# TaceoLabs/collaborative-circom

Hardware: AMD Instinct MI355X
Metric: Groth16 constraints/sec (BN254, 2^22 R1CS), one REP3 party's prove (higher is better)
Workload: dtype u32; 1 GPU; synthetic R1CS 2^22 constraints-domain BN254, REP3 co-groth16 (configs[2]); num_constraints=4194302, domain_size=4194304, nnz=12582906, msm=8 G1 + 2 G2 of ~2^22 points, ntt=12

## Files before the change

collaborative-circom_amd/csrc/capi_internal.hpp:

```cpp
#pragma once
#include "common.hpp"
#include "launchers.hpp"
#include "curve.hpp"
#include "subgroup.hpp"
#include "host_ec64.hpp"
#include "ntt_kernels.hpp"
#include "plonk_kernels.hpp"

#include <cmath>
#include <chrono>
#include <map>
#include <set>
#include <mutex>
#include <vector>

using namespace cg;

hipError_t hip_malloc_flush(void** p, size_t bytes);
template <class T> hipError_t hip_malloc_flush(T** p, size_t bytes) { return hip_malloc_flush((void**)p, bytes); }

namespace cgi {

struct Arena {
    char* base = nullptr; size_t cap = 0, used = 0;
    void* take(size_t bytes) { void* p = base + used; used += align_up(bytes); return p; }
};

enum { TW_BITREV = 1, TW_NATURAL = 2 };
struct TwKey { int curve; int log_m; uint32_t gen[8]; int kind = 0;
    bool operator<(const TwKey& o) const { if (curve != o.curve) return curve < o.curve; if (log_m != o.log_m) return log_m < o.log_m; if (kind != o.kind) return kind < o.kind; return memcmp(gen, o.gen, sizeof gen) < 0; } };
struct CosetKey { TwKey k; uint32_t scale[8]; bool operator<(const CosetKey& o) const { if (k < o.k) return true; if (o.k < k) return false; return memcmp(scale, o.scale, sizeof scale) < 0; } };
struct CosetTables { void* lo; void* hi; int log_lo; };

enum { TAG_MSM = 0, TAG_NTT, TAG_VEC, TAG_SPMV, TAG_SORT, TAG_ACC_G1, TAG_ACC_G2, TAG_REDUCE, TAG_COUNT };
struct EvPair { hipEvent_t a, b; int tag; };

struct MsmFold { enum { WINDOWS = 0, PLAIN = 1, BITS = 2, GRID = 3 }; int kind = WINDOWS, c = 0, nsums = 0, log_l = 0, log_h = 0; uint32_t gc = 1, gr = 1; };

struct MsmTicket {
    bool live = false;
    int curve = 0, group = 0, k = 0, c = 0, nwin = 0;
    uint32_t* h_flags = nullptr; bool optimistic = false;
    const cg_bases* bases = nullptr; size_t offset = 0, n = 0; std::vector<const void*> scalars;
    int nsums = 0;
    MsmFold fold;
    void* h_pinned = nullptr; size_t pinned_bytes = 0;
    hipEvent_t done = nullptr;
};

}
using namespace cgi;


// ... 166 lines not shown
```

collaborative-circom_amd/csrc/capi_ntt.hip:

```cpp
#include "capi_internal.hpp"

namespace {
template <class Fr>
void host_pow_tables(const Fr& w, const Fr& first, int log_lo, size_t hi_n, std::vector<Fr>& lo, std::vector<Fr>& hi) {
    lo.resize((size_t)1 << log_lo); hi.resize(hi_n);
    Fr acc = first, step = Fr::one();
    for (size_t j = 0; j < lo.size(); j++) { lo[j] = acc; acc = acc * w; step = step * w; }
    Fr h = Fr::one();
    for (size_t j = 0; j < hi_n; j++) { hi[j] = h; h = h * step; }
}

struct SharedTwiddles { void* p; size_t bytes; int refs; uint64_t stamp; };
std::mutex g_tw_mu;
std::map<std::pair<int, TwKey>, SharedTwiddles> g_tw;
uint64_t g_tw_clock = 0;
void* shared_twiddles_acquire(int device, const TwKey& key) {
    std::lock_guard<std::mutex> l(g_tw_mu);
    auto it = g_tw.find({device, key});
    if (it == g_tw.end()) return nullptr;
    it->second.refs++; it->second.stamp = ++g_tw_clock;
    return it->second.p;
}
void* shared_twiddles_publish(int device, const TwKey& key, void* p, size_t bytes) {
    std::lock_guard<std::mutex> l(g_tw_mu);
// ... 4 lines not shown
}
}
void shared_twiddles_release(int device, const TwKey& key) {
    std::lock_guard<std::mutex> l(g_tw_mu);
    auto it = g_tw.find({device, key});
    if (it != g_tw.end() && it->second.refs > 0) it->second.refs--;
    for (;;) {
        size_t idle = 0; auto victim = g_tw.end();
        for (auto j = g_tw.begin(); j != g_tw.end(); ++j) if (j->second.refs == 0) { idle += j->second.bytes; if (victim == g_tw.end() || j->second.stamp < victim->second.stamp) victim = j; }
        if (idle <= ((size_t)1 << 30) || victim == g_tw.end()) break;
        hipFree(victim->second.p); g_tw.erase(victim);
    }
}
namespace {

template <class Fr> Fr mont32() { Fr c = Fr::one(); for (int i = 0; i < 5; i++) c = c + c; return c; }
template <class Fr> Fr inv_pow2(int log_m) {
    uint32_t e[Fr::N] = {0}; e[log_m / 32] = 1u << (log_m % 32);
    Fr nn; for (int i = 0; i < Fr::N; i++) nn.v[i] = e[i];
    return fp_inverse(nn.to_mont());
}

template <class Fr>
int get_twiddles_lazy(cg_ctx* ctx, int curve, int log_m, const Fr& w, bool natural, const void** out) {
    TwKey key; key.curve = curve; key.log_m = log_m; key.kind = natural ? TW_NATURAL : TW_BITREV; memcpy(key.gen, w.v, sizeof key.gen);
    auto it = ctx->twiddles.find(key);
    if (it != ctx->twiddles.end()) { *out = it->second; return 0; }
    if (void* shared = shared_twiddles_acquire(ctx->device, key)) { ctx->twiddles[key] = shared; *out = shared; return 0; }
    const size_t m = (size_t)1 << log_m;
    const int log_lo = std::min(11, std::max(0, log_m - 1));
    const size_t hi_n = std::max<size_t>(1, (m / 2) >> log_lo);
    std::vector<Fr> lo, hi;
    host_pow_tables(w, Fr::one(), log_lo, hi_n, lo, hi);
    Fr *d_lo = nullptr, *d_hi = nullptr; void* d_tw = nullptr;
    const size_t bytes = lazy29_bytes(std::max<size_t>(m / 2, 1));
    HIPCHK(hip_malloc_flush((void**)&d_lo, lo.size() * sizeof(Fr)));
    HIPCHK(hip_malloc_flush((void**)&d_hi, hi.size() * sizeof(Fr)));
    HIPCHK(hip_malloc_flush(&d_tw, bytes));
    HIPCHK(hipMemcpyAsync(d_lo, lo.data(), lo.size() * sizeof(Fr), hipMemcpyHostToDevice, ctx->stream));
    HIPCHK(hipMemcpyAsync(d_hi, hi.data(), hi.size() * sizeof(Fr), hipMemcpyHostToDevice, ctx->stream));
    {
        const int rc = natural ? launch_build_twiddles_lazy_natural<Fr>(ctx->stream, d_tw, m, d_lo, d_hi, log_lo, mont32<Fr>())
                               : launch_build_twiddles_lazy<Fr>(ctx->stream, d_tw, m, log_m, d_lo, d_hi, log_lo, mont32<Fr>());
        if (rc) return rc;
    }
    HIPCHK(hipStreamSynchronize(ctx->stream));
    HIPCHK(hipFree(d_lo)); HIPCHK(hipFree(d_hi));
    d_tw = shared_twiddles_publish(ctx->device, key, d_tw, bytes);
    ctx->twiddles[key] = d_tw;
    *out = d_tw;
    return 0;
}

template <class Fr>
int get_coset_tables(cg_ctx* ctx, int curve, int log_m, const Fr& g, const Fr& scale, CosetTables* out) {
    CosetKey key; key.k.curve = curve; key.k.log_m = log_m; memcpy(key.k.gen, g.v, sizeof key.k.gen); memcpy(key.scale, scale.v, sizeof key.scale);
    auto it = ctx->cosets.find(key);
    if (it != ctx->cosets.end()) { *out = it->second; return 0; }
    const size_t m = (size_t)1 << log_m;
    const int log_lo = std::min(11, log_m);
    const size_t hi_n = std::max<size_t>(1, m >> log_lo);
    std::vector<Fr> lo, hi;
    host_pow_tables(g, scale, log_lo, hi_n, lo, hi);
    CosetTables t; t.log_lo = log_lo;
    HIPCHK(hip_malloc_flush(&t.lo, lo.size() * sizeof(Fr)));
    HIPCHK(hip_malloc_flush(&t.hi, hi.size() * sizeof(Fr)));
    HIPCHK(hipMemcpy(t.lo, lo.data(), lo.size() * sizeof(Fr), hipMemcpyHostToDevice));
    HIPCHK(hipMemcpy(t.hi, hi.data(), hi.size() * sizeof(Fr), hipMemcpyHostToDevice));
    if (ctx->cosets.size() >= 64) {
        HIPCHK(hipStreamSynchronize(ctx->stream));
// ... 17 lines not shown
            int k = rest / np + (i < rest % np ? 1 : 0);
            plan.push_back({s0, k, tile_log - k});
            s0 += k;
        }
    }
    plan.push_back({s0, k_last, 0});
    return plan;
}

int ntt_lazy_tile() {
    static const int tile = [] { const char* e = tune_env("CG_NTT_TILE"); const int v = e ? atoi(e) : NTT_TILE_LOG_LAZY; return std::min(NTT_TILE_LOG, std::max(8, v)); }();
    return tile;
}

template <class Fr>
int ntt_run(cg_ctx* ctx, int curve, void* const* d_vecs, int k, size_t n, const Fr& gen, bool inverse, const Fr* coset, size_t arena_off) {
    const int log_m = log2_floor(n);
    if (((size_t)1 << log_m) != n) return fail(CG_ERR_ARG, "NTT length must be a power of two");
    if (k < 1 || k > NTT_MAX_VECS) return fail(CG_ERR_ARG, "k out of range");
    if (n == 1) return 0;
    if (!inverse && coset) return fail(CG_ERR_ARG, "coset_gen is only supported with inverse != 0");
    const Fr w = inverse ? fp_inverse(gen) : gen;
    const void* twl = nullptr;
    int rc = get_twiddles_lazy<Fr>(ctx, curve, log_m, w, false, &twl);
    if (rc) return rc;
    NttVecs data{}, tmp{};
    for (int j = 0; j < k; j++) { data.p[j] = d_vecs[j]; tmp.p[j] = ctx->ntt_arena.base + arena_off + (size_t)j * lazy29_bytes(n); }
    hipStream_t st = ctx->stream;
    bool first = true;
    for (const NttPass& p : ntt_plan(log_m, ntt_lazy_tile())) { rc = launch_ntt_ct_pass<Fr>(st, first, first ? data : tmp, tmp, k, n, log_m, p.s0, p.k, p.t, twl); if (rc) return rc; first = false; }
    const Fr scale32 = inverse ? mont32<Fr>() * inv_pow2<Fr>(log_m) : mont32<Fr>();
    CosetTables t;
    const Fr* d_scale = nullptr; const Fr* c_lo = nullptr; const Fr* c_hi = nullptr; int log_lo = 0;
    if (coset) { rc = get_coset_tables<Fr>(ctx, curve, log_m, *coset, scale32, &t); if (rc) return rc; c_lo = (const Fr*)t.lo; c_hi = (const Fr*)t.hi; log_lo = t.log_lo; }
    else { rc = get_coset_tables<Fr>(ctx, curve, 0, Fr::one(), scale32, &t); if (rc) return rc; d_scale = (const Fr*)t.lo; }
    return launch_bitrev_finish_lazy<Fr>(st, data, tmp, k, n, log_m, d_scale, c_lo, c_hi, log_lo);
}

template <class Fr>
int ntt_coset_pair_run(cg_ctx* ctx, int curve, void* const* d_vecs, int k, size_t n, const Fr& gen, const Fr& coset, size_t arena_off) {
    const int log_m = log2_floor(n);
    if (((size_t)1 << log_m) != n) return fail(CG_ERR_ARG, "NTT length must be a power of two");
    if (k < 1 || k > NTT_MAX_VECS) return fail(CG_ERR_ARG, "k out of range");
    if (n == 1) return 0;
    const void* tw_inv = nullptr; const void* tw_fwd = nullptr;
    int rc = get_twiddles_lazy<Fr>(ctx, curve, log_m, fp_inverse(gen), false, &tw_inv); if (rc) return rc;
    rc = get_twiddles_lazy<Fr>(ctx, curve, log_m, gen, true, &tw_fwd); if (rc) return rc;
    const Fr c32 = mont32<Fr>();
    CosetTables ct;
    rc = get_coset_tables<Fr>(ctx, curve, log_m, coset, c32 * inv_pow2<Fr>(log_m), &ct); if (rc) return rc;
    NttVecs data{}, tmp{};
    for (int j = 0; j < k; j++) { data.p[j] = d_vecs[j]; tmp.p[j] = ctx->ntt_arena.base + arena_off + (size_t)j * lazy29_bytes(n); }
    hipStream_t st = ctx->stream;
    const std::vector<NttPass> plan = ntt_plan(log_m, ntt_lazy_tile());
    bool first = true;
    for (const NttPass& p : plan) { rc = launch_ntt_ct_pass<Fr>(st, first, first ? data : tmp, tmp, k, n, log_m, p.s0, p.k, p.t, tw_inv); if (rc) return rc; first = false; }
    for (size_t i = plan.size(); i-- > 0;) {
        const NttPass& p = plan[i];
        rc = launch_ntt_dit_pass<Fr>(st, i + 1 == plan.size(), i == 0, data, tmp, k, n, log_m, p.s0, p.k, p.t, tw_fwd, (const Fr*)ct.lo, (const Fr*)ct.hi, ct.log_lo, c32);
        if (rc) return rc;
    }
    return 0;
}

}

extern "C" {
int32_t cg_ntt_dev(cg_ctx* ctx, int32_t curve, void* const* d_vecs, int32_t k, size_t n, const void* h_group_gen, int32_t inverse, const void* h_coset_gen) {
    if (!ctx || !d_vecs || !h_group_gen) return fail(CG_ERR_ARG, "null argument");
    HIPCHK(hipSetDevice(ctx->device));
    return with_fr(curve, [&](auto tag) -> int {
        typedef decltype(tag) Fr;
        Fr gen, cos; copy_in(gen, h_group_gen);
        if (h_coset_gen) copy_in(cos, h_coset_gen);
        if (n > 1) { int rc = ensure_ntt_arena(ctx, (size_t)k * lazy29_bytes(n)); if (rc) return rc; }
        StatScope ss(ctx, TAG_NTT);
        return ntt_run<Fr>(ctx, curve, d_vecs, k, n, gen, inverse != 0, h_coset_gen ? &cos : nullptr, 0);
    });
}
int32_t cg_ntt_coset_pair_dev(cg_ctx* ctx, int32_t curve, void* const* d_vecs, int32_t k, size_t n, const void* h_group_gen, const void* h_coset_gen) {
    if (!ctx || !d_vecs || !h_group_gen || !h_coset_gen) return fail(CG_ERR_ARG, "null argument");
    HIPCHK(hipSetDevice(ctx->device));
// ... 38 lines not shown
```

collaborative-circom_amd/csrc/fr_impl.hpp:

```cpp
#pragma once
#include "launchers.hpp"
#include "ntt_kernels.hpp"
#include "vec_kernels.hpp"
#include "plonk_kernels.hpp"
#include "r1cs_kernels.hpp"
#include "plonk_setup_kernels.hpp"
#include "msm_sort_kernels.hpp"

namespace cg {

template <class Fr> int launch_vec_binary(hipStream_t st, int op, Fr* out, const Fr* a, const Fr* b, size_t n) {
    if (!n) return 0;
    if (op == 0) hipLaunchKernelGGL((k_vec_binary<Fr, 0>), dim3(grid_for(n)), dim3(256), 0, st, out, a, b, n);
    else if (op == 1) hipLaunchKernelGGL((k_vec_binary<Fr, 1>), dim3(grid_for(n)), dim3(256), 0, st, out, a, b, n);
    else hipLaunchKernelGGL((k_vec_binary<Fr, 2>), dim3(grid_for(n)), dim3(256), 0, st, out, a, b, n);
    HIPCHK(hipGetLastError());
    return 0;
}
template <class Fr> int launch_rep3_mul_local(hipStream_t st, Fr* out, const Fr* aa, const Fr* ab, const Fr* ba, const Fr* bb, const Fr* mask, size_t n) {
    if (!n) return 0;
    hipLaunchKernelGGL((k_rep3_mul_local<Fr>), dim3(grid_for(n)), dim3(256), 0, st, out, aa, ab, ba, bb, mask, n);
    HIPCHK(hipGetLastError());
    return 0;
}
// ... 151 lines not shown
template <class Fr> int launch_plonk_sigma_labels(hipStream_t st, const uint32_t* prev, const Fr* wpow, int log_n, const Fr& k1, const Fr& k2, Fr* sigma) {
    hipLaunchKernelGGL((k_plonk_sigma_labels<Fr>), dim3(grid_for((size_t)3 << log_n)), dim3(256), 0, st, prev, wpow, log_n, k1, k2, sigma);
    HIPCHK(hipGetLastError());
    return 0;
}
template <class Fr> int launch_build_twiddles_lazy(hipStream_t st, void* tw, size_t m, int log_m, const Fr* lo, const Fr* hi, int log_lo, const Fr& c32) {
    if (m > 1) hipLaunchKernelGGL((k_build_twiddles_lazy<Fr>), dim3(grid_for(m / 2)), dim3(256), 0, st, tw, m / 2, log_m, lo, hi, log_lo, c32);
    HIPCHK(hipGetLastError());
    return 0;
}
template <class Fr> int launch_ntt_ct_pass(hipStream_t st, bool first, NttVecs src, NttVecs dst, int nvec, size_t n, int log_m, int s0, int k, int t, const void* tw) {
    static PerDeviceOnce attr_set;
    if (attr_set.pending()) {
        HIPCHK(hipFuncSetAttribute((const void*)k_ntt_ct_pass<Fr, true>, hipFuncAttributeMaxDynamicSharedMemorySize, 36 << NTT_TILE_LOG));
        HIPCHK(hipFuncSetAttribute((const void*)k_ntt_ct_pass<Fr, false>, hipFuncAttributeMaxDynamicSharedMemorySize, 36 << NTT_TILE_LOG));
        attr_set.mark();
    }
    const int E = 1 << (k + t);
    if (first) hipLaunchKernelGGL((k_ntt_ct_pass<Fr, true>), dim3((unsigned)(n / E), nvec), dim3(NTT_THREADS), (size_t)E * 36, st, src, dst, log_m, s0, k, t, tw);
    else hipLaunchKernelGGL((k_ntt_ct_pass<Fr, false>), dim3((unsigned)(n / E), nvec), dim3(NTT_THREADS), (size_t)E * 36, st, src, dst, log_m, s0, k, t, tw);
    HIPCHK(hipGetLastError());
    return 0;
}
template <class Fr> int launch_build_twiddles_lazy_natural(hipStream_t st, void* tw, size_t m, const Fr* lo, const Fr* hi, int log_lo, const Fr& c32) {
    if (m > 1) hipLaunchKernelGGL((k_build_twiddles_lazy_natural<Fr>), dim3(grid_for(m / 2)), dim3(256), 0, st, tw, m / 2, lo, hi, log_lo, c32);
    HIPCHK(hipGetLastError());
    return 0;
}
template <class Fr> int launch_ntt_dit_pass(hipStream_t st, bool first, bool last, NttVecs out, NttVecs tmp, int nvec, size_t n, int log_m, int s0, int k, int t, const void* tw,
                                            const Fr* c_lo, const Fr* c_hi, int log_lo, const Fr& c32) {
    static PerDeviceOnce attr_set;
    if (attr_set.pending()) {
        HIPCHK(hipFuncSetAttribute((const void*)k_ntt_dit_pass<Fr, true, true>, hipFuncAttributeMaxDynamicSharedMemorySize, 36 << NTT_TILE_LOG));
        HIPCHK(hipFuncSetAttribute((const void*)k_ntt_dit_pass<Fr, true, false>, hipFuncAttributeMaxDynamicSharedMemorySize, 36 << NTT_TILE_LOG));
        HIPCHK(hipFuncSetAttribute((const void*)k_ntt_dit_pass<Fr, false, true>, hipFuncAttributeMaxDynamicSharedMemorySize, 36 << NTT_TILE_LOG));
        HIPCHK(hipFuncSetAttribute((const void*)k_ntt_dit_pass<Fr, false, false>, hipFuncAttributeMaxDynamicSharedMemorySize, 36 << NTT_TILE_LOG));
        attr_set.mark();
    }
    const int E = 1 << (k + t);
    const dim3 grid((unsigned)(n / E), nvec); const size_t lds = (size_t)E * 36;
    if (first && last) hipLaunchKernelGGL((k_ntt_dit_pass<Fr, true, true>), grid, dim3(NTT_THREADS), lds, st, out, tmp, log_m, s0, k, t, tw, c_lo, c_hi, log_lo, c32);
    else if (first) hipLaunchKernelGGL((k_ntt_dit_pass<Fr, true, false>), grid, dim3(NTT_THREADS), lds, st, out, tmp, log_m, s0, k, t, tw, c_lo, c_hi, log_lo, c32);
    else if (last) hipLaunchKernelGGL((k_ntt_dit_pass<Fr, false, true>), grid, dim3(NTT_THREADS), lds, st, out, tmp, log_m, s0, k, t, tw, c_lo, c_hi, log_lo, c32);
    else hipLaunchKernelGGL((k_ntt_dit_pass<Fr, false, false>), grid, dim3(NTT_THREADS), lds, st, out, tmp, log_m, s0, k, t, tw, c_lo, c_hi, log_lo, c32);
    HIPCHK(hipGetLastError());
    return 0;
}
template <class Fr> int launch_bitrev_finish_lazy(hipStream_t st, NttVecs dst, NttVecs src, int nvec, size_t n, int log_m, const Fr* scale, const Fr* c_lo, const Fr* c_hi, int log_lo) {
    if (log_m >= 2 * BITREV_B_LAZY)
        hipLaunchKernelGGL((k_bitrev_finish_lazy<Fr>), dim3((unsigned)(n >> (2 * BITREV_B_LAZY)), nvec), dim3(256), 0, st, dst, src, log_m, scale, c_lo, c_hi, log_lo);
    else
        hipLaunchKernelGGL((k_bitrev_finish_lazy_small<Fr>), dim3(grid_for(n), nvec), dim3(256), 0, st, dst, src, log_m, scale, c_lo, c_hi, log_lo);
    HIPCHK(hipGetLastError());
    return 0;
}

inline bool msm_sort_use_partition(size_t n, int c, int nwin, int shared, bool any_size = false) {
    const size_t nbuckets = (size_t)(shared ? 1 : nwin) << (c - 1);
    const size_t nregions = (nbuckets + ((size_t)1 << PART_REGION_LOG) - 1) >> PART_REGION_LOG;
    return (any_size || (size_t)nwin * n >= ((size_t)1 << 21)) && nregions >= 8 && nregions <= PART_MAX_REGIONS;
}
template <class Fr> int msm_sort_launch(hipStream_t st, const Fr* d_scalars, size_t n, int c, int nwin, int shared, char* scratch, size_t scratch_bytes, MsmSortPtrs* out, hipEvent_t* evs,
                                        int force) {
    if (force != 0 && force != CG_MSM_PATH_GENERAL && force != CG_MSM_PATH_SMALL && force != CG_MSM_PATH_PARTITION) return fail(CG_ERR_ARG, "msm_sort_launch: not a path of the dense schedule");
    const size_t nbuckets = (size_t)(shared ? 1 : nwin) << (c - 1);
    size_t off = 0;
    auto take = [&](size_t bytes) { void* p = scratch + off; off += align_up(bytes); return p; };
// ... 119 lines not shown
    template decltype(launch_vec_gather_strided<Fr>) launch_vec_gather_strided<Fr>;                                        \
    template decltype(launch_vec_lincomb<Fr>) launch_vec_lincomb<Fr>;                                                      \
    template decltype(launch_shamir_share<Fr>) launch_shamir_share<Fr>;                                                    \
    template decltype(launch_plonk_r2_factors<Fr>) launch_plonk_r2_factors<Fr>;                                            \
    template decltype(launch_prefix_scan<Fr>) launch_prefix_scan<Fr>;                                                      \
    template decltype(launch_vec_inverse<Fr>) launch_vec_inverse<Fr>;                                                      \
    template decltype(launch_plonk_additions<Fr>) launch_plonk_additions<Fr>;                                              \
    template decltype(launch_plonk_r3_blind<Fr>) launch_plonk_r3_blind<Fr>;                                                \
    template decltype(launch_plonk_r3_perm<Fr>) launch_plonk_r3_perm<Fr>;                                                  \
    template decltype(launch_plonk_r3_gate<Fr>) launch_plonk_r3_gate<Fr>;                                                  \
    template decltype(launch_plonk_mul4_tail<Fr>) launch_plonk_mul4_tail<Fr>;                                              \
    template decltype(launch_plonk_r3_t<Fr>) launch_plonk_r3_t<Fr>;                                                        \
    template decltype(launch_plonk_r3_divide<Fr>) launch_plonk_r3_divide<Fr>;                                              \
    template decltype(launch_plonk_gate_check<Fr>) launch_plonk_gate_check<Fr>;                                            \
    template decltype(launch_vec_mismatch<Fr>) launch_vec_mismatch<Fr>;                                                    \
    template decltype(launch_spmv_csr<Fr>) launch_spmv_csr<Fr>;                                                            \
    template decltype(launch_r1cs_check<Fr>) launch_r1cs_check<Fr>;                                                        \
    template decltype(launch_qap_columns<Fr>) launch_qap_columns<Fr>;                                                      \
    template decltype(launch_plonk_gate_count<Fr>) launch_plonk_gate_count<Fr>;                                            \
    template decltype(launch_plonk_gate_emit<Fr>) launch_plonk_gate_emit<Fr>;                                              \
    template decltype(launch_plonk_sigma_labels<Fr>) launch_plonk_sigma_labels<Fr>;                                        \
    template decltype(launch_build_twiddles_lazy<Fr>) launch_build_twiddles_lazy<Fr>;                                      \
    template decltype(launch_ntt_ct_pass<Fr>) launch_ntt_ct_pass<Fr>;                                                      \
    template decltype(launch_build_twiddles_lazy_natural<Fr>) launch_build_twiddles_lazy_natural<Fr>;                      \
    template decltype(launch_ntt_dit_pass<Fr>) launch_ntt_dit_pass<Fr>;                                                    \
    template decltype(launch_bitrev_finish_lazy<Fr>) launch_bitrev_finish_lazy<Fr>;                                        \
    template decltype(msm_sort_launch<Fr>) msm_sort_launch<Fr>;                                                            \
    template decltype(msm_sort_direct_launch<Fr>) msm_sort_direct_launch<Fr>;                                              \
    }
```

collaborative-circom_amd/csrc/launchers.hpp:

```cpp
#pragma once
#include "common.hpp"

namespace cg {

template <class F> struct Affine;
template <class F> struct XYZZ;
template <class F> struct FastSubgroup;
struct NttVecs;
template <class F> struct PlonkR2Args;
template <class F> struct PlonkBlindArgs;
template <class F> struct PlonkPermArgs;
template <class F> struct PlonkGateArgs;
template <class F> struct PlonkMul4Args;
template <class F> struct PlonkTArgs;
template <class F> struct PlonkDivArgs;
template <class F> struct PlonkCheckArgs;

constexpr int SCAN_TILE = 2048;
constexpr int PART_TILE = 16384;
constexpr int PART_REGION_LOG = 9;
constexpr int PART_MAX_REGIONS = 4096;
struct MsmSortPtrs { const uint32_t* sorted; const uint32_t* offsets; const uint32_t* counts; uint32_t cap; const uint32_t* overflow; int path; };
inline size_t msm_sort_scratch_bytes(size_t n, int c, int nwin) {
    const size_t nbuckets = (size_t)nwin << (c - 1);
// ... 49 lines not shown
template <class Fr> int launch_qap_columns(hipStream_t st, const uint32_t* col_ptr, const uint32_t* row, const Fr* coeff, size_t n_cols, const Fr* L, Fr* out, uint32_t long_min);
struct PlonkGateOut {
    uint32_t* map[3];
    void* q[5];
    uint32_t* add_ids;
    void* add_f;
};
template <class Fr> int launch_plonk_gate_count(hipStream_t st, const R1csMat& A, const R1csMat& B, const R1csMat& C, size_t n_rows, uint32_t* counts, uint32_t* offsets, uint32_t* tile_sums);
template <class Fr> int launch_plonk_gate_emit(hipStream_t st, const R1csMat& A, const R1csMat& B, const R1csMat& C, size_t n_rows, uint32_t n_wires, uint32_t n_public,
                                               const uint32_t* counts, const uint32_t* offsets, size_t n_constraints, size_t n, const PlonkGateOut& o);
template <class Fr> int launch_plonk_sigma_labels(hipStream_t st, const uint32_t* prev, const Fr* wpow, int log_n, const Fr& k1, const Fr& k2, Fr* sigma);
template <class Fr> int launch_plonk_additions(hipStream_t st, const uint32_t* order, size_t n, const uint32_t* ids, const Fr* coeffs, const Fr* pub, uint32_t n_inputs, int pc,
                                               Fr* ext_a, Fr* ext_b, size_t n_priv);
template <class Fr> int launch_plonk_r2_factors(hipStream_t st, const PlonkR2Args<Fr>& g, size_t n);
template <class Fr> int launch_plonk_r3_blind(hipStream_t st, const PlonkBlindArgs<Fr>& g, size_t n);
template <class Fr> int launch_plonk_r3_perm(hipStream_t st, const PlonkPermArgs<Fr>& g, size_t n);
template <class Fr> int launch_plonk_r3_gate(hipStream_t st, const PlonkGateArgs<Fr>& g, size_t n);
template <class Fr> int launch_plonk_mul4_tail(hipStream_t st, const PlonkMul4Args<Fr>& g, size_t n);
template <class Fr> int launch_plonk_r3_t(hipStream_t st, const PlonkTArgs<Fr>& g, size_t n);
template <class Fr> int launch_plonk_r3_divide(hipStream_t st, const PlonkDivArgs<Fr>& g, size_t n);
template <class Fr> int launch_plonk_gate_check(hipStream_t st, const PlonkCheckArgs<Fr>& g, size_t n, unsigned long long* result);
template <class Fr> int launch_vec_mismatch(hipStream_t st, const Fr* a, size_t a_stride, const Fr* b, size_t b_stride, size_t first, size_t n, unsigned long long* result);
template <class Fr> int launch_build_twiddles_lazy(hipStream_t st, void* tw, size_t m, int log_m, const Fr* lo, const Fr* hi, int log_lo, const Fr& c32);
template <class Fr> int launch_build_twiddles_lazy_natural(hipStream_t st, void* tw, size_t m, const Fr* lo, const Fr* hi, int log_lo, const Fr& c32);
template <class Fr> int launch_ntt_ct_pass(hipStream_t st, bool first, NttVecs src, NttVecs dst, int nvec, size_t n, int log_m, int s0, int k, int t, const void* tw);
template <class Fr> int launch_ntt_dit_pass(hipStream_t st, bool first, bool last, NttVecs out, NttVecs tmp, int nvec, size_t n, int log_m, int s0, int k, int t, const void* tw,
                                            const Fr* c_lo, const Fr* c_hi, int log_lo, const Fr& c32);
template <class Fr> int launch_bitrev_finish_lazy(hipStream_t st, NttVecs dst, NttVecs src, int nvec, size_t n, int log_m, const Fr* scale, const Fr* c_lo, const Fr* c_hi, int log_lo);

int chacha12_fr_rand_launch(hipStream_t st, const uint32_t* key8, const uint32_t* mod8, int modulus_bits, uint64_t word_pos, uint64_t n_pairs, uint64_t n,
                            void* d_cand, uint32_t* d_tiles, unsigned long long* d_result, void* d_out);

}
```

collaborative-circom_amd/csrc/ntt_kernels.hpp:

```cpp
#pragma once
#include "field.hpp"
#include "lazy29.hpp"
#include "vec_kernels.hpp"

namespace cg {

constexpr int NTT_MAX_VECS = 8;
struct NttVecs { void* p[NTT_MAX_VECS]; };

constexpr int NTT_TILE_LOG = 11;
constexpr int NTT_THREADS = 256;
constexpr int NTT_TILE_LOG_LAZY = 10;
constexpr int BITREV_B_LAZY = 5;

struct Lazy29Planes { uint4* p0; uint4* p1; uint32_t* p2; };
__host__ __device__ inline size_t lazy29_bytes(size_t n) { return ((n * 36 + 255) / 256) * 256; }
__device__ __forceinline__ Lazy29Planes lazy29_planes(void* base, size_t n) {
    char* b = reinterpret_cast<char*>(base);
    return {reinterpret_cast<uint4*>(b), reinterpret_cast<uint4*>(b + n * 16), reinterpret_cast<uint32_t*>(b + n * 32)};
}
template <class L> __device__ __forceinline__ L lazy29_load(const uint4* p0, const uint4* p1, const uint32_t* p2, size_t i) {
    const uint4 x = p0[i], y = p1[i]; L r;
    r.l[0] = (int32_t)x.x; r.l[1] = (int32_t)x.y; r.l[2] = (int32_t)x.z; r.l[3] = (int32_t)x.w;
    r.l[4] = (int32_t)y.x; r.l[5] = (int32_t)y.y; r.l[6] = (int32_t)y.z; r.l[7] = (int32_t)y.w; r.l[8] = (int32_t)p2[i];
// ... 70 lines not shown
    for (; q < k; q++) {
        const int pb = k - 1 - q;
        for (int u = threadIdx.x; u < E / 2; u += NTT_THREADS) {
            const int lo_local = u & tmask;
            const int mu = u >> t;
            const int mid0 = ((mu >> pb) << (pb + 1)) | (mu & ((1 << pb) - 1));
            const int i0 = (mid0 << t) | lo_local;
            const int i1 = i0 + (1 << (pb + t));
            const size_t blk = (hi << q) | (size_t)(mid0 >> (k - q));
            const L a = lazy29_load<L>(pl0, pl1, pl2, i0), b = lazy29_load<L>(pl0, pl1, pl2, i1);
            const L w = lazy29_load<L>(tw.p0, tw.p1, tw.p2, blk);
            const L v = L::mul_cols(b, w);
            lazy29_store<L>(pl0, pl1, pl2, i0, (a + v).norm());
            lazy29_store<L>(pl0, pl1, pl2, i1, (a - v).norm());
        }
        __syncthreads();
    }
    for (int idx = threadIdx.x; idx < E; idx += NTT_THREADS) {
        const size_t g = base + ((size_t)(idx >> t) << lo_bits) + (idx & tmask);
        lazy29_store<L>(dst.p0, dst.p1, dst.p2, g, lazy29_load<L>(pl0, pl1, pl2, idx));
    }
}

template <class F>
__global__ void __launch_bounds__(256) k_build_twiddles_lazy_natural(void* tw_base, size_t half, const F* __restrict__ lo, const F* __restrict__ hi, int log_lo, F c32) {
    typedef L29<F> L;
    const Lazy29Planes tw = lazy29_planes(tw_base, half);
    for (size_t e = (size_t)blockIdx.x * blockDim.x + threadIdx.x; e < half; e += (size_t)gridDim.x * blockDim.x) {
        const F w = ld_fp(lo + (e & (((size_t)1 << log_lo) - 1))) * ld_fp(hi + (e >> log_lo)) * c32;
        lazy29_store<L>(tw.p0, tw.p1, tw.p2, e, L::template unpack<0>(w));
    }
}
template <class F, bool FIRST, bool LAST>
__global__ void __launch_bounds__(NTT_THREADS) k_ntt_dit_pass(NttVecs out_vecs, NttVecs tmp_vecs, int log_m, int s0, int k, int t, const void* tw_base,
                                                             const F* __restrict__ cos_lo, const F* __restrict__ cos_hi, int log_lo, F c32) {
    static_assert(F::N == 8, "NTT is specialised for 256-bit scalar fields");
    typedef L29<F> L;
    extern __shared__ uint4 lds[];
    const int E = 1 << (k + t);
    uint4* pl0 = lds;
    uint4* pl1 = lds + E;
    uint32_t* pl2 = reinterpret_cast<uint32_t*>(lds + 2 * E);
    const size_t m = (size_t)1 << log_m;
    const Lazy29Planes tw = lazy29_planes(const_cast<void*>(tw_base), m / 2);
    const Lazy29Planes buf = lazy29_planes(tmp_vecs.p[blockIdx.y], m);
    const int lo_bits = log_m - s0 - k;
    const size_t tiles_per_hi = (size_t)1 << (lo_bits - t);
    const size_t hi = blockIdx.x / tiles_per_hi;
    const size_t lo0 = (blockIdx.x % tiles_per_hi) << t;
    const size_t base = (hi << (log_m - s0)) + lo0;
    const int tmask = (1 << t) - 1;

    for (int idx = threadIdx.x; idx < E; idx += NTT_THREADS) {
        const size_t g = base + ((size_t)(idx >> t) << lo_bits) + (idx & tmask);
        L v = lazy29_load<L>(buf.p0, buf.p1, buf.p2, g);
        if constexpr (FIRST) {
            const size_t i = (size_t)(__brevll((unsigned long long)g) >> (64 - log_m));
            const F c = ld_fp(cos_lo + (i & (((size_t)1 << log_lo) - 1))) * ld_fp(cos_hi + (i >> log_lo));
            v = L::mul_cols(v, L::template unpack<0>(c));
        }
        lazy29_store<L>(pl0, pl1, pl2, idx, v);
    }
    __syncthreads();
    int q = 0;
    for (; q + 1 < k; q += 2) {
        const int s = lo_bits + q;
        for (int u = threadIdx.x; u < E / 4; u += NTT_THREADS) {
            const int lo_local = u & tmask;
            const int mu = u >> t;
            const int mid0 = ((mu >> q) << (q + 2)) | (mu & ((1 << q) - 1));
            const int i00 = (mid0 << t) | lo_local, d = 1 << (q + t);
            const size_t j = ((size_t)(mid0 & ((1 << q) - 1)) << lo_bits) + lo0 + lo_local;
            const size_t e0 = j << (log_m - 1 - s), e1 = j << (log_m - 2 - s);
            const L a00 = lazy29_load<L>(pl0, pl1, pl2, i00), a01 = lazy29_load<L>(pl0, pl1, pl2, i00 + d);
            const L a10 = lazy29_load<L>(pl0, pl1, pl2, i00 + 2 * d), a11 = lazy29_load<L>(pl0, pl1, pl2, i00 + 3 * d);
            const L w0 = lazy29_load<L>(tw.p0, tw.p1, tw.p2, e0);
            L v1, v3; L::mul2_cols(a01, w0, a11, w0, v1, v3);
            const L b00 = a00 + v1, b01 = a00 - v1;
            const L b10 = (a10 + v3).norm(), b11 = (a10 - v3).norm();
            const L w1a = lazy29_load<L>(tw.p0, tw.p1, tw.p2, e1), w1b = lazy29_load<L>(tw.p0, tw.p1, tw.p2, e1 + (m >> 2));
            L y2, y3; L::mul2_cols(b10, w1a, b11, w1b, y2, y3);
            lazy29_store<L>(pl0, pl1, pl2, i00, (b00 + y2).norm());
            lazy29_store<L>(pl0, pl1, pl2, i00 + 2 * d, (b00 - y2).norm());
            lazy29_store<L>(pl0, pl1, pl2, i00 + d, (b01 + y3).norm());
            lazy29_store<L>(pl0, pl1, pl2, i00 + 3 * d, (b01 - y3).norm());
        }
        __syncthreads();
    }
    for (; q < k; q++) {
        const int s = lo_bits + q;
        for (int u = threadIdx.x; u < E / 2; u += NTT_THREADS) {
            const int lo_local = u & tmask;
            const int mu = u >> t;
            const int mid0 = ((mu >> q) << (q + 1)) | (mu & ((1 << q) - 1));
            const int i0 = (mid0 << t) | lo_local, i1 = i0 + (1 << (q + t));
            const size_t j = ((size_t)(mid0 & ((1 << q) - 1)) << lo_bits) + lo0 + lo_local;
            const L a = lazy29_load<L>(pl0, pl1, pl2, i0), b = lazy29_load<L>(pl0, pl1, pl2, i1);
            const L v = L::mul_cols(b, lazy29_load<L>(tw.p0, tw.p1, tw.p2, j << (log_m - 1 - s)));
            lazy29_store<L>(pl0, pl1, pl2, i0, (a + v).norm());
            lazy29_store<L>(pl0, pl1, pl2, i1, (a - v).norm());
        }
        __syncthreads();
    }
    for (int idx = threadIdx.x; idx < E; idx += NTT_THREADS) {
        const size_t g = base + ((size_t)(idx >> t) << lo_bits) + (idx & tmask);
        const L v = lazy29_load<L>(pl0, pl1, pl2, idx);
        if constexpr (LAST) st_fp(reinterpret_cast<F*>(out_vecs.p[blockIdx.y]) + g, L::pack_reduced(L::mul_cols(v, L::template unpack<0>(c32))));
        else lazy29_store<L>(buf.p0, buf.p1, buf.p2, g, v);
    }
}

template <class F>
__global__ void __launch_bounds__(256) k_bitrev_finish_lazy(NttVecs dst, NttVecs src, int log_m, const F* __restrict__ scale,
                                                            const F* __restrict__ cos_lo, const F* __restrict__ cos_hi, int log_lo) {
    typedef L29<F> L;
    constexpr int B = BITREV_B_LAZY, S = 1 << B;
    __shared__ uint4 tile0[S * (S + 1)];
    __shared__ uint4 tile1[S * (S + 1)];
    __shared__ uint32_t tile2[S * (S + 1)];
    const size_t m = (size_t)1 << log_m;
    const Lazy29Planes in = lazy29_planes(src.p[blockIdx.y], m);
    F* out = reinterpret_cast<F*>(dst.p[blockIdx.y]);
    const int mid_bits = log_m - 2 * B;
    const size_t mid = blockIdx.x;
    const size_t rmid = mid_bits > 0 ? (__brevll((unsigned long long)mid) >> (64 - mid_bits)) : 0;
    for (int e = threadIdx.x; e < S * S; e += 256) {
        const int h = e >> B, l = e & (S - 1);
        const size_t i = ((size_t)h << (log_m - B)) | (mid << B) | (size_t)l;
        tile0[h * (S + 1) + l] = in.p0[i]; tile1[h * (S + 1) + l] = in.p1[i]; tile2[h * (S + 1) + l] = in.p2[i];
    }
// ... 27 lines not shown
```

Baseline: 61.85 million constraints/s.

## Fold coset scaling into per-stage forward NTT twiddles

Precomputes a stage-indexed twiddle table in which each stage's twiddles absorb the matching power of the coset generator. The forward DIT pass therefore no longer does a per-element coset multiply on its first pass, and the bit-reversed coset table lookups go away. In exchange the forward twiddle table doubles in size. For domains too large for the lazy-reduction bound, the code falls back to separate inverse-coset and forward NTT runs.

```diff
diff --git a/collaborative-circom_amd/csrc/capi_internal.hpp b/collaborative-circom_amd/csrc/capi_internal.hpp
--- a/collaborative-circom_amd/csrc/capi_internal.hpp
+++ b/collaborative-circom_amd/csrc/capi_internal.hpp
@@ -26,9 +26,11 @@
     void* take(size_t bytes) { void* p = base + used; used += align_up(bytes); return p; }
 };
 
-enum { TW_BITREV = 1, TW_NATURAL = 2 };
+enum { TW_BITREV = 1, TW_COSET_STAGES = 2 };
 struct TwKey { int curve; int log_m; uint32_t gen[8]; int kind = 0;
-    bool operator<(const TwKey& o) const { if (curve != o.curve) return curve < o.curve; if (log_m != o.log_m) return log_m < o.log_m; if (kind != o.kind) return kind < o.kind; return memcmp(gen, o.gen, sizeof gen) < 0; } };
+    uint32_t coset[8] = {0};
+    bool operator<(const TwKey& o) const { if (curve != o.curve) return curve < o.curve; if (log_m != o.log_m) return log_m < o.log_m; if (kind != o.kind) return kind < o.kind;
+                                           const int c = memcmp(gen, o.gen, sizeof gen); return c ? c < 0 : memcmp(coset, o.coset, sizeof coset) < 0; } };
 struct CosetKey { TwKey k; uint32_t scale[8]; bool operator<(const CosetKey& o) const { if (k < o.k) return true; if (o.k < k) return false; return memcmp(scale, o.scale, sizeof scale) < 0; } };
 struct CosetTables { void* lo; void* hi; int log_lo; };
 
diff --git a/collaborative-circom_amd/csrc/capi_ntt.hip b/collaborative-circom_amd/csrc/capi_ntt.hip
--- a/collaborative-circom_amd/csrc/capi_ntt.hip
+++ b/collaborative-circom_amd/csrc/capi_ntt.hip
@@ -50,30 +50,40 @@
 }
 
 template <class Fr>
-int get_twiddles_lazy(cg_ctx* ctx, int curve, int log_m, const Fr& w, bool natural, const void** out) {
-    TwKey key; key.curve = curve; key.log_m = log_m; key.kind = natural ? TW_NATURAL : TW_BITREV; memcpy(key.gen, w.v, sizeof key.gen);
+int get_twiddles_lazy(cg_ctx* ctx, int curve, int log_m, const Fr& w, const Fr* coset, const void** out) {
+    TwKey key; key.curve = curve; key.log_m = log_m; key.kind = coset ? TW_COSET_STAGES : TW_BITREV; memcpy(key.gen, w.v, sizeof key.gen);
+    if (coset) memcpy(key.coset, coset->v, sizeof key.coset);
     auto it = ctx->twiddles.find(key);
     if (it != ctx->twiddles.end()) { *out = it->second; return 0; }
     if (void* shared = shared_twiddles_acquire(ctx->device, key)) { ctx->twiddles[key] = shared; *out = shared; return 0; }
     const size_t m = (size_t)1 << log_m;
     const int log_lo = std::min(11, std::max(0, log_m - 1));
     const size_t hi_n = std::max<size_t>(1, (m / 2) >> log_lo);
-    std::vector<Fr> lo, hi;
+    std::vector<Fr> lo, hi, gpow32;
     host_pow_tables(w, Fr::one(), log_lo, hi_n, lo, hi);
-    Fr *d_lo = nullptr, *d_hi = nullptr; void* d_tw = nullptr;
-    const size_t bytes = lazy29_bytes(std::max<size_t>(m / 2, 1));
+    if (coset) {
+        gpow32.resize(log_m);
+        Fr p = *coset;
+        for (int s = log_m - 1; s >= 0; s--) { gpow32[s] = p * mont32<Fr>(); p = p * p; }
+    }
+    Fr *d_lo = nullptr, *d_hi = nullptr, *d_gpow = nullptr; void* d_tw = nullptr;
+    const size_t bytes = lazy29_bytes(coset ? m : std::max<size_t>(m / 2, 1));
     HIPCHK(hip_malloc_flush((void**)&d_lo, lo.size() * sizeof(Fr)));
     HIPCHK(hip_malloc_flush((void**)&d_hi, hi.size() * sizeof(Fr)));
     HIPCHK(hip_malloc_flush(&d_tw, bytes));
     HIPCHK(hipMemcpyAsync(d_lo, lo.data(), lo.size() * sizeof(Fr), hipMemcpyHostToDevice, ctx->stream));
     HIPCHK(hipMemcpyAsync(d_hi, hi.data(), hi.size() * sizeof(Fr), hipMemcpyHostToDevice, ctx->stream));
+    if (coset) {
+        HIPCHK(hip_malloc_flush((void**)&d_gpow, gpow32.size() * sizeof(Fr)));
+        HIPCHK(hipMemcpyAsync(d_gpow, gpow32.data(), gpow32.size() * sizeof(Fr), hipMemcpyHostToDevice, ctx->stream));
+    }
     {
-        const int rc = natural ? launch_build_twiddles_lazy_natural<Fr>(ctx->stream, d_tw, m, d_lo, d_hi, log_lo, mont32<Fr>())
-                               : launch_build_twiddles_lazy<Fr>(ctx->stream, d_tw, m, log_m, d_lo, d_hi, log_lo, mont32<Fr>());
+        const int rc = coset ? launch_build_twiddles_lazy_coset_stages<Fr>(ctx->stream, d_tw, m, log_m, d_lo, d_hi, log_lo, d_gpow)
+                             : launch_build_twiddles_lazy<Fr>(ctx->stream, d_tw, m, log_m, d_lo, d_hi, log_lo, mont32<Fr>());
         if (rc) return rc;
     }
     HIPCHK(hipStreamSynchronize(ctx->stream));
-    HIPCHK(hipFree(d_lo)); HIPCHK(hipFree(d_hi));
+    HIPCHK(hipFree(d_lo)); HIPCHK(hipFree(d_hi)); if (d_gpow) HIPCHK(hipFree(d_gpow));
     d_tw = shared_twiddles_publish(ctx->device, key, d_tw, bytes);
     ctx->twiddles[key] = d_tw;
     *out = d_tw;
@@ -137,7 +147,7 @@
     if (!inverse && coset) return fail(CG_ERR_ARG, "coset_gen is only supported with inverse != 0");
     const Fr w = inverse ? fp_inverse(gen) : gen;
     const void* twl = nullptr;
-    int rc = get_twiddles_lazy<Fr>(ctx, curve, log_m, w, false, &twl);
+    int rc = get_twiddles_lazy<Fr>(ctx, curve, log_m, w, nullptr, &twl);
     if (rc) return rc;
     NttVecs data{}, tmp{};
     for (int j = 0; j < k; j++) { data.p[j] = d_vecs[j]; tmp.p[j] = ctx->ntt_arena.base + arena_off + (size_t)j * lazy29_bytes(n); }
@@ -158,12 +168,14 @@
     if (((size_t)1 << log_m) != n) return fail(CG_ERR_ARG, "NTT length must be a power of two");
     if (k < 1 || k > NTT_MAX_VECS) return fail(CG_ERR_ARG, "k out of range");
     if (n == 1) return 0;
+    if (log_m > ntt_pair_max_log<Fr>()) {
+        const int rc = ntt_run<Fr>(ctx, curve, d_vecs, k, n, gen, true, &coset, arena_off);
+        return rc ? rc : ntt_run<Fr>(ctx, curve, d_vecs, k, n, gen, false, nullptr, arena_off);
+    }
     const void* tw_inv = nullptr; const void* tw_fwd = nullptr;
-    int rc = get_twiddles_lazy<Fr>(ctx, curve, log_m, fp_inverse(gen), false, &tw_inv); if (rc) return rc;
-    rc = get_twiddles_lazy<Fr>(ctx, curve, log_m, gen, true, &tw_fwd); if (rc) return rc;
-    const Fr c32 = mont32<Fr>();
-    CosetTables ct;
-    rc = get_coset_tables<Fr>(ctx, curve, log_m, coset, c32 * inv_pow2<Fr>(log_m), &ct); if (rc) return rc;
+    int rc = get_twiddles_lazy<Fr>(ctx, curve, log_m, fp_inverse(gen), nullptr, &tw_inv); if (rc) return rc;
+    rc = get_twiddles_lazy<Fr>(ctx, curve, log_m, gen, &coset, &tw_fwd); if (rc) return rc;
+    const Fr c_last = mont32<Fr>() * inv_pow2<Fr>(log_m);
     NttVecs data{}, tmp{};
     for (int j = 0; j < k; j++) { data.p[j] = d_vecs[j]; tmp.p[j] = ctx->ntt_arena.base + arena_off + (size_t)j * lazy29_bytes(n); }
     hipStream_t st = ctx->stream;
@@ -172,7 +184,7 @@
     for (const NttPass& p : plan) { rc = launch_ntt_ct_pass<Fr>(st, first, first ? data : tmp, tmp, k, n, log_m, p.s0, p.k, p.t, tw_inv); if (rc) return rc; first = false; }
     for (size_t i = plan.size(); i-- > 0;) {
         const NttPass& p = plan[i];
-        rc = launch_ntt_dit_pass<Fr>(st, i + 1 == plan.size(), i == 0, data, tmp, k, n, log_m, p.s0, p.k, p.t, tw_fwd, (const Fr*)ct.lo, (const Fr*)ct.hi, ct.log_lo, c32);
+        rc = launch_ntt_dit_pass<Fr>(st, i == 0, data, tmp, k, n, log_m, p.s0, p.k, p.t, tw_fwd, c_last);
         if (rc) return rc;
     }
     return 0;
diff --git a/collaborative-circom_amd/csrc/fr_impl.hpp b/collaborative-circom_amd/csrc/fr_impl.hpp
--- a/collaborative-circom_amd/csrc/fr_impl.hpp
+++ b/collaborative-circom_amd/csrc/fr_impl.hpp
@@ -197,27 +197,22 @@
     HIPCHK(hipGetLastError());
     return 0;
 }
-template <class Fr> int launch_build_twiddles_lazy_natural(hipStream_t st, void* tw, size_t m, const Fr* lo, const Fr* hi, int log_lo, const Fr& c32) {
-    if (m > 1) hipLaunchKernelGGL((k_build_twiddles_lazy_natural<Fr>), dim3(grid_for(m / 2)), dim3(256), 0, st, tw, m / 2, lo, hi, log_lo, c32);
-    HIPCHK(hipGetLastError());
-    return 0;
-}
-template <class Fr> int launch_ntt_dit_pass(hipStream_t st, bool first, bool last, NttVecs out, NttVecs tmp, int nvec, size_t n, int log_m, int s0, int k, int t, const void* tw,
-                                            const Fr* c_lo, const Fr* c_hi, int log_lo, const Fr& c32) {
+template <class Fr> int launch_build_twiddles_lazy_coset_stages(hipStream_t st, void* tw, size_t m, int log_m, const Fr* lo, const Fr* hi, int log_lo, const Fr* gpow32) {
+    if (m > 1) hipLaunchKernelGGL((k_build_twiddles_lazy_coset_stages<Fr>), dim3(grid_for(m)), dim3(256), 0, st, tw, m, log_m, lo, hi, log_lo, gpow32);
+    HIPCHK(hipGetLastError());
+    return 0;
+}
+template <class Fr> int launch_ntt_dit_pass(hipStream_t st, bool last, NttVecs out, NttVecs tmp, int nvec, size_t n, int log_m, int s0, int k, int t, const void* tw, const Fr& c_last) {
     static PerDeviceOnce attr_set;
     if (attr_set.pending()) {
-        HIPCHK(hipFuncSetAttribute((const void*)k_ntt_dit_pass<Fr, true, true>, hipFuncAttributeMaxDynamicSharedMemorySize, 36 << NTT_TILE_LOG));
-        HIPCHK(hipFuncSetAttribute((const void*)k_ntt_dit_pass<Fr, true, false>, hipFuncAttributeMaxDynamicSharedMemorySize, 36 << NTT_TILE_LOG));
-        HIPCHK(hipFuncSetAttribute((const void*)k_ntt_dit_pass<Fr, false, true>, hipFuncAttributeMaxDynamicSharedMemorySize, 36 << NTT_TILE_LOG));
-        HIPCHK(hipFuncSetAttribute((const void*)k_ntt_dit_pass<Fr, false, false>, hipFuncAttributeMaxDynamicSharedMemorySize, 36 << NTT_TILE_LOG));
+        HIPCHK(hipFuncSetAttribute((const void*)k_ntt_dit_pass<Fr, true>, hipFuncAttributeMaxDynamicSharedMemorySize, 36 << NTT_TILE_LOG));
+        HIPCHK(hipFuncSetAttribute((const void*)k_ntt_dit_pass<Fr, false>, hipFuncAttributeMaxDynamicSharedMemorySize, 36 << NTT_TILE_LOG));
         attr_set.mark();
     }
     const int E = 1 << (k + t);
     const dim3 grid((unsigned)(n / E), nvec); const size_t lds = (size_t)E * 36;
-    if (first && last) hipLaunchKernelGGL((k_ntt_dit_pass<Fr, true, true>), grid, dim3(NTT_THREADS), lds, st, out, tmp, log_m, s0, k, t, tw, c_lo, c_hi, log_lo, c32);
-    else if (first) hipLaunchKernelGGL((k_ntt_dit_pass<Fr, true, false>), grid, dim3(NTT_THREADS), lds, st, out, tmp, log_m, s0, k, t, tw, c_lo, c_hi, log_lo, c32);
-    else if (last) hipLaunchKernelGGL((k_ntt_dit_pass<Fr, false, true>), grid, dim3(NTT_THREADS), lds, st, out, tmp, log_m, s0, k, t, tw, c_lo, c_hi, log_lo, c32);
-    else hipLaunchKernelGGL((k_ntt_dit_pass<Fr, false, false>), grid, dim3(NTT_THREADS), lds, st, out, tmp, log_m, s0, k, t, tw, c_lo, c_hi, log_lo, c32);
+    if (last) hipLaunchKernelGGL((k_ntt_dit_pass<Fr, true>), grid, dim3(NTT_THREADS), lds, st, out, tmp, log_m, s0, k, t, tw, c_last);
+    else hipLaunchKernelGGL((k_ntt_dit_pass<Fr, false>), grid, dim3(NTT_THREADS), lds, st, out, tmp, log_m, s0, k, t, tw, c_last);
     HIPCHK(hipGetLastError());
     return 0;
 }
@@ -383,7 +378,7 @@
     template decltype(launch_plonk_sigma_labels<Fr>) launch_plonk_sigma_labels<Fr>;                                        \
     template decltype(launch_build_twiddles_lazy<Fr>) launch_build_twiddles_lazy<Fr>;                                      \
     template decltype(launch_ntt_ct_pass<Fr>) launch_ntt_ct_pass<Fr>;                                                      \
-    template decltype(launch_build_twiddles_lazy_natural<Fr>) launch_build_twiddles_lazy_natural<Fr>;                      \
+    template decltype(launch_build_twiddles_lazy_coset_stages<Fr>) launch_build_twiddles_lazy_coset_stages<Fr>;            \
     template decltype(launch_ntt_dit_pass<Fr>) launch_ntt_dit_pass<Fr>;                                                    \
     template decltype(launch_bitrev_finish_lazy<Fr>) launch_bitrev_finish_lazy<Fr>;                                        \
     template decltype(msm_sort_launch<Fr>) msm_sort_launch<Fr>;                                                            \
diff --git a/collaborative-circom_amd/csrc/launchers.hpp b/collaborative-circom_amd/csrc/launchers.hpp
--- a/collaborative-circom_amd/csrc/launchers.hpp
+++ b/collaborative-circom_amd/csrc/launchers.hpp
@@ -95,10 +95,9 @@
 template <class Fr> int launch_plonk_gate_check(hipStream_t st, const PlonkCheckArgs<Fr>& g, size_t n, unsigned long long* result);
 template <class Fr> int launch_vec_mismatch(hipStream_t st, const Fr* a, size_t a_stride, const Fr* b, size_t b_stride, size_t first, size_t n, unsigned long long* result);
 template <class Fr> int launch_build_twiddles_lazy(hipStream_t st, void* tw, size_t m, int log_m, const Fr* lo, const Fr* hi, int log_lo, const Fr& c32);
-template <class Fr> int launch_build_twiddles_lazy_natural(hipStream_t st, void* tw, size_t m, const Fr* lo, const Fr* hi, int log_lo, const Fr& c32);
+template <class Fr> int launch_build_twiddles_lazy_coset_stages(hipStream_t st, void* tw, size_t m, int log_m, const Fr* lo, const Fr* hi, int log_lo, const Fr* gpow32);
 template <class Fr> int launch_ntt_ct_pass(hipStream_t st, bool first, NttVecs src, NttVecs dst, int nvec, size_t n, int log_m, int s0, int k, int t, const void* tw);
-template <class Fr> int launch_ntt_dit_pass(hipStream_t st, bool first, bool last, NttVecs out, NttVecs tmp, int nvec, size_t n, int log_m, int s0, int k, int t, const void* tw,
-                                            const Fr* c_lo, const Fr* c_hi, int log_lo, const Fr& c32);
+template <class Fr> int launch_ntt_dit_pass(hipStream_t st, bool last, NttVecs out, NttVecs tmp, int nvec, size_t n, int log_m, int s0, int k, int t, const void* tw, const Fr& c_last);
 template <class Fr> int launch_bitrev_finish_lazy(hipStream_t st, NttVecs dst, NttVecs src, int nvec, size_t n, int log_m, const Fr* scale, const Fr* c_lo, const Fr* c_hi, int log_lo);
 
 int chacha12_fr_rand_launch(hipStream_t st, const uint32_t* key8, const uint32_t* mod8, int modulus_bits, uint64_t word_pos, uint64_t n_pairs, uint64_t n,
diff --git a/collaborative-circom_amd/csrc/ntt_kernels.hpp b/collaborative-circom_amd/csrc/ntt_kernels.hpp
--- a/collaborative-circom_amd/csrc/ntt_kernels.hpp
+++ b/collaborative-circom_amd/csrc/ntt_kernels.hpp
@@ -116,18 +116,32 @@
     }
 }
 
-template <class F>
-__global__ void __launch_bounds__(256) k_build_twiddles_lazy_natural(void* tw_base, size_t half, const F* __restrict__ lo, const F* __restrict__ hi, int log_lo, F c32) {
-    typedef L29<F> L;
-    const Lazy29Planes tw = lazy29_planes(tw_base, half);
-    for (size_t e = (size_t)blockIdx.x * blockDim.x + threadIdx.x; e < half; e += (size_t)gridDim.x * blockDim.x) {
-        const F w = ld_fp(lo + (e & (((size_t)1 << log_lo) - 1))) * ld_fp(hi + (e >> log_lo)) * c32;
-        lazy29_store<L>(tw.p0, tw.p1, tw.p2, e, L::template unpack<0>(w));
-    }
-}
-template <class F, bool FIRST, bool LAST>
-__global__ void __launch_bounds__(NTT_THREADS) k_ntt_dit_pass(NttVecs out_vecs, NttVecs tmp_vecs, int log_m, int s0, int k, int t, const void* tw_base,
-                                                             const F* __restrict__ cos_lo, const F* __restrict__ cos_hi, int log_lo, F c32) {
+template <class F> constexpr int ntt_pair_max_log() {
+    const double R = 137438953472.0  / ((double)F::Params::P[F::N - 1] + 1.0);
+    int log_m = 0;
+    for (double b = 1.0;; log_m++) {
+        b = b * (1.0 + 1.0 / R) + 1.0; b = b * (1.0 + 1.0 / R) + 1.0;
+        if (!(b < R)) return log_m;
+    }
+}
+template <class F>
+__global__ void __launch_bounds__(256) k_build_twiddles_lazy_coset_stages(void* tw_base, size_t m, int log_m, const F* __restrict__ lo, const F* __restrict__ hi, int log_lo,
+                                                                         const F* __restrict__ gpow32) {
+    typedef L29<F> L;
+    const Lazy29Planes tw = lazy29_planes(tw_base, m);
+    for (size_t i = (size_t)blockIdx.x * blockDim.x + threadIdx.x; i < m; i += (size_t)gridDim.x * blockDim.x) {
+        L v;
+        if (i == 0) { _Pragma("unroll") for (int k = 0; k < L::NL; k++) v.l[k] = 0; }
+        else {
+            const int s = 63 - __clzll((unsigned long long)i);
+            const size_t e = (i - ((size_t)1 << s)) << (log_m - 1 - s);
+            v = L::template unpack<0>(ld_fp(lo + (e & (((size_t)1 << log_lo) - 1))) * ld_fp(hi + (e >> log_lo)) * ld_fp(gpow32 + s));
+        }
+        lazy29_store<L>(tw.p0, tw.p1, tw.p2, i, v);
+    }
+}
+template <class F, bool LAST>
+__global__ void __launch_bounds__(NTT_THREADS) k_ntt_dit_pass(NttVecs out_vecs, NttVecs tmp_vecs, int log_m, int s0, int k, int t, const void* tw_base, F c_last) {
     static_assert(F::N == 8, "NTT is specialised for 256-bit scalar fields");
     typedef L29<F> L;
     extern __shared__ uint4 lds[];
@@ -136,7 +150,7 @@
     uint4* pl1 = lds + E;
     uint32_t* pl2 = reinterpret_cast<uint32_t*>(lds + 2 * E);
     const size_t m = (size_t)1 << log_m;
-    const Lazy29Planes tw = lazy29_planes(const_cast<void*>(tw_base), m / 2);
+    const Lazy29Planes tw = lazy29_planes(const_cast<void*>(tw_base), m);
     const Lazy29Planes buf = lazy29_planes(tmp_vecs.p[blockIdx.y], m);
     const int lo_bits = log_m - s0 - k;
     const size_t tiles_per_hi = (size_t)1 << (lo_bits - t);
@@ -147,13 +161,7 @@
 
     for (int idx = threadIdx.x; idx < E; idx += NTT_THREADS) {
         const size_t g = base + ((size_t)(idx >> t) << lo_bits) + (idx & tmask);
-        L v = lazy29_load<L>(buf.p0, buf.p1, buf.p2, g);
-        if constexpr (FIRST) {
-            const size_t i = (size_t)(__brevll((unsigned long long)g) >> (64 - log_m));
-            const F c = ld_fp(cos_lo + (i & (((size_t)1 << log_lo) - 1))) * ld_fp(cos_hi + (i >> log_lo));
-            v = L::mul_cols(v, L::template unpack<0>(c));
-        }
-        lazy29_store<L>(pl0, pl1, pl2, idx, v);
+        lazy29_store<L>(pl0, pl1, pl2, idx, lazy29_load<L>(buf.p0, buf.p1, buf.p2, g));
     }
     __syncthreads();
     int q = 0;
@@ -165,14 +173,14 @@
             const int mid0 = ((mu >> q) << (q + 2)) | (mu & ((1 << q) - 1));
             const int i00 = (mid0 << t) | lo_local, d = 1 << (q + t);
             const size_t j = ((size_t)(mid0 & ((1 << q) - 1)) << lo_bits) + lo0 + lo_local;
-            const size_t e0 = j << (log_m - 1 - s), e1 = j << (log_m - 2 - s);
+            const size_t e0 = ((size_t)1 << s) + j, e1 = ((size_t)2 << s) + j;
             const L a00 = lazy29_load<L>(pl0, pl1, pl2, i00), a01 = lazy29_load<L>(pl0, pl1, pl2, i00 + d);
             const L a10 = lazy29_load<L>(pl0, pl1, pl2, i00 + 2 * d), a11 = lazy29_load<L>(pl0, pl1, pl2, i00 + 3 * d);
             const L w0 = lazy29_load<L>(tw.p0, tw.p1, tw.p2, e0);
             L v1, v3; L::mul2_cols(a01, w0, a11, w0, v1, v3);
             const L b00 = a00 + v1, b01 = a00 - v1;
             const L b10 = (a10 + v3).norm(), b11 = (a10 - v3).norm();
-            const L w1a = lazy29_load<L>(tw.p0, tw.p1, tw.p2, e1), w1b = lazy29_load<L>(tw.p0, tw.p1, tw.p2, e1 + (m >> 2));
+            const L w1a = lazy29_load<L>(tw.p0, tw.p1, tw.p2, e1), w1b = lazy29_load<L>(tw.p0, tw.p1, tw.p2, e1 + ((size_t)1 << s));
             L y2, y3; L::mul2_cols(b10, w1a, b11, w1b, y2, y3);
             lazy29_store<L>(pl0, pl1, pl2, i00, (b00 + y2).norm());
             lazy29_store<L>(pl0, pl1, pl2, i00 + 2 * d, (b00 - y2).norm());
@@ -190,7 +198,7 @@
             const int i0 = (mid0 << t) | lo_local, i1 = i0 + (1 << (q + t));
             const size_t j = ((size_t)(mid0 & ((1 << q) - 1)) << lo_bits) + lo0 + lo_local;
             const L a = lazy29_load<L>(pl0, pl1, pl2, i0), b = lazy29_load<L>(pl0, pl1, pl2, i1);
-            const L v = L::mul_cols(b, lazy29_load<L>(tw.p0, tw.p1, tw.p2, j << (log_m - 1 - s)));
+            const L v = L::mul_cols(b, lazy29_load<L>(tw.p0, tw.p1, tw.p2, ((size_t)1 << s) + j));
             lazy29_store<L>(pl0, pl1, pl2, i0, (a + v).norm());
             lazy29_store<L>(pl0, pl1, pl2, i1, (a - v).norm());
         }
@@ -199,7 +207,7 @@
     for (int idx = threadIdx.x; idx < E; idx += NTT_THREADS) {
         const size_t g = base + ((size_t)(idx >> t) << lo_bits) + (idx & tmask);
         const L v = lazy29_load<L>(pl0, pl1, pl2, idx);
-        if constexpr (LAST) st_fp(reinterpret_cast<F*>(out_vecs.p[blockIdx.y]) + g, L::pack_reduced(L::mul_cols(v, L::template unpack<0>(c32))));
+        if constexpr (LAST) st_fp(reinterpret_cast<F*>(out_vecs.p[blockIdx.y]) + g, L::pack_reduced(L::mul_cols(v, L::template unpack<0>(c_last))));
         else lazy29_store<L>(buf.p0, buf.p1, buf.p2, g, v);
     }
 }
```

Result: no change. 62.37 million constraints/s (median of 6 runs) (+0.8%).
